# legend-exp/dspeed

Measured on AMD Instinct MI355X. Metric: waveforms/sec, 4096-sample fp32 trap-energy chain, higher is better.
Workload: dtype f32; 1 GPU; 1000000 x 4096 float32 rows per GPU, fused bl_subtract->pole_zero(tau=1716.28)->trap_filter(625,188)->fixed_time_pickoff('l'); BASELINE configs[1]; rows_per_gpu=1000000, wf_len=4096, device= (gfx950:sramecc+:xnack-), entry=build_processing_chain, kernel=dsp_energy_rr_kernel, lds_bytes_per_wave=19696, waves_per_block=4, blocks=512

## Files before the change

### dspeed_amd/csrc/dsp_energy.hip

```cpp
#include <hip/hip_runtime.h>

#include "dsp_program.h"
#include "dsp_wave.h"

struct EnergyArgs {
    const void* wf;
    int64_t wf_stride;
    int32_t wf_offset;
    int32_t len;
    const float* bl;
    int64_t bl_stride;
    float bl_const;
    int32_t has_bl;
    const float* tp;
    int64_t tp_stride;
    float tp_const;
    int32_t mode;
    float* out;
    int64_t out_stride;
    double c;
    double rr, ll;
    int32_t tau_nan;
    int32_t all_nan;
    int32_t C, pitch;
// ... 258 lines not shown
                        if (t + 2 * G3 < C) fetch(a0, a1, a2, a3, t + 2 * G3);
                        body(b0, b1, b2, b3, t + G3);
                    }
                }
                PHASE(4)
                const double D = (double)y - (double)g;
                const double delta = wave_exscan_add(D) - (double)g;
                float w4[4];
#pragma unroll
                for (int k = 0; k < 4; ++k) {
                    const float v = (float)((double)capv[k] + delta);
                    w4[k] = cl[k] >= 0 ? readlane(v, cl[k]) : 0.0f;
                }
                int fc = 0;
                result = pickoff_eval(t_in, A.mode, len, w4, fc);
                if (fc) report(fc, row);
            }
        }
        if (lane == 0) A.out[row * A.out_stride] = result;
        wave_sync();
        PHASE(5)
    }
    if (stamps && lane == 0) {
#pragma unroll
        for (int i = 0; i < 6; ++i) atomicAdd(reinterpret_cast<unsigned long long*>(err + 4) + i, tsum[i]);
    }
}

struct EnergyPlan {
    int32_t shift[3][4];
    int32_t cs[3][4];
    int32_t local[3][4];
};

__device__ __attribute__((noinline)) double rr_decay(double tau) { return exp(-1.0 / tau); }

template <int NPF, int KIND, int S, int IN, bool TAU = false>
__global__ void __launch_bounds__(256, NPF >= 32 ? 1 : 2) dsp_energy_rr_kernel(EnergyArgs A, EnergyPlan PL, int64_t n_wf, int* err) {
    extern __shared__ __attribute__((aligned(16))) unsigned char smem_raw[];
    constexpr int C = 4 * NPF + 1, len = 256 * NPF, NG = (C - 1) / 8, CS = (C - 1) / S, NGS = CS / 8;
    constexpr int BS = CS >= 16 ? 16 : CS;
    static_assert((C - 1) % (8 * S) == 0, "sub-chain length must be a whole number of 8-sample groups");
    const int lane = lane_id();
    const double inv_rr = 1.0 / A.rr, inv_ll = 1.0 / A.ll;
    const int wave = __builtin_amdgcn_readfirstlane((int)(threadIdx.x >> 6)), wpb = (int)(blockDim.x >> 6);
    float* lds = reinterpret_cast<float*>(smem_raw) + (size_t)wave * A.lds_elems_per_wave;
    for (int e = lane; e < A.lds_elems_per_wave; e += 64) lds[e] = 0.0f;
    wave_sync();
    float* slot = lds + A.slot_off;
    float* mine = slot + lane * C;
    constexpr int AUXP = NG + 1 <= 9 ? 9 : ((NG + 1) | 1);
    static_assert(NG + 1 <= AUXP && S * NGS + 1 <= AUXP && (AUXP & 1) == 1, "side array too small");
    float* aux = slot + 64 * C + 16 + lane * AUXP;
    const float* lagp[3];
#pragma unroll
    for (int k = 0; k < 3; ++k) {
        const int pos0 = lane * C - A.q[k];
        lagp[k] = (pos0 >= -C) ? slot + pos0 : slot - (2 * C + 8);
    }

    const int64_t stride_rows = (int64_t)gridDim.x * wpb;
    int64_t row = (int64_t)blockIdx.x * wpb + wave;
    typedef float f4 __attribute__((ext_vector_type(4)));
    typedef unsigned int u4 __attribute__((ext_vector_type(4)));
    constexpr int NLD = IN == 0 ? NPF : NPF / 2;
    static_assert(IN == 0 || NPF % 2 == 0, "16-bit rows: an even number of 4-sample groups per lane");
    u4 pf[NLD];
    float pf_bl = 0.0f, pf_tp = 0.0f;
    auto prefetch = [&](int64_t r) {
        const char* g = (const char*)A.wf + (r * A.wf_stride + A.wf_offset) * (IN == 0 ? 4 : 2);
#pragma unroll
        for (int b = 0; b < NLD; ++b) pf[b] = reinterpret_cast<const u4*>(g)[b * 64 + lane];
        typedef const __attribute__((address_space(1))) float* gptr;
        pf_bl = A.bl ? ((gptr)A.bl)[r * A.bl_stride] : A.bl_const;
        pf_tp = A.tp ? ((gptr)A.tp)[r * A.tp_stride] : A.tp_const;
    };
    auto report = [&](int code, int64_t r) {
        if (lane == 0 && atomicCAS(&err[0], 0, code) == 0) {
            err[1] = (int)(r & 0xffffffffll);
            err[2] = (int)(r >> 32);
        }
    };
    if (row < n_wf) prefetch(row);
    const bool stamps = (ABLATE(A) & 8) != 0;
    unsigned long long tsum[6] = {0, 0, 0, 0, 0, 0}, tlast = stamps ? stamp() : 0;
    float pend_result = 0.0f;
    int64_t pend_row = -1;

    for (; row < n_wf; row += stride_rows) {
#pragma unroll
        for (int b = 0; b < NLD; ++b) {
            if (IN == 0) {
                f4 v;
#pragma unroll
                for (int m = 0; m < 4; ++m) v[m] = __uint_as_float(pf[b][m]);
                *reinterpret_cast<f4*>(slot + (b * 64 + lane) * 4) = v - pf_bl;
            } else {
                f4 lo, hi;
#pragma unroll
                for (int m = 0; m < 4; ++m) {
                    const unsigned int wv = pf[b][m];
                    const float s0 = IN == 1 ? (float)(short)(wv & 0xffffu) : (float)(wv & 0xffffu);
                    const float s1 = IN == 1 ? (float)(short)(wv >> 16) : (float)(wv >> 16);
                    if (m < 2) {
                        lo[2 * m] = s0;
                        lo[2 * m + 1] = s1;
                    } else {
                        hi[2 * (m - 2)] = s0;
                        hi[2 * (m - 2) + 1] = s1;
                    }
                }
                *reinterpret_cast<f4*>(slot + (b * 64 + lane) * 8) = lo - pf_bl;
                *reinterpret_cast<f4*>(slot + (b * 64 + lane) * 8 + 4) = hi - pf_bl;
            }
        }
        slot[len + lane] = 0.0f;
        const float t_in = __int_as_float(__builtin_amdgcn_readfirstlane(__float_as_int(pf_tp)));
        const int64_t next = row + stride_rows;
        __builtin_amdgcn_sched_barrier(0);
        if (next < n_wf) prefetch(next);
        if (pend_row >= 0 && lane == 0) A.out[pend_row * A.out_stride] = pend_result;
        __builtin_amdgcn_sched_barrier(0);
        wave_sync();
        PHASE(0)
        RR_PRIO_AT(0)

        float result = quiet_nan<float>();
        float xr[C];
#pragma unroll
        for (int t = 0; t < C; ++t) xr[t] = mine[t];
        const float xprev = (lane > 0) ? mine[-1] : 0.0f;
        double Xp[4] = {0.0, 0.0, 0.0, 0.0};
#pragma unroll
        for (int t = 0; t < C; ++t) {
            if ((t & 7) == 0) __builtin_amdgcn_sched_barrier(0);
            Xp[t & 3] += (double)xr[t];
        }
        const double X = (Xp[0] + Xp[1]) + (Xp[2] + Xp[3]);
        double c_row = A.c;
        bool in_nan = A.tau_nan != 0;
        if constexpr (TAU) {
            const float tau = A.tau[row * A.tau_stride];
            in_nan = tau != tau;
            c_row = rr_decay((double)tau);
        }
        if (wave_any(!(fabs(X) <= 1.7976931348623157e308))) {
            bool n = false;
#pragma unroll
            for (int t = 0; t < C; ++t) n |= (xr[t] != xr[t]);
            in_nan |= wave_any(n);
        }
        PHASE(1)
        RR_PRIO_AT(1)
#pragma unroll
        for (int t = 0; t < C; ++t) asm volatile("" : "+v"(xr[t]));
        if (!in_nan) {
            const double E = wave_exscan_add(X);
            const double c = c_row;
            double xp = (double)xprev, acc = E - c * (E - xp);
            float run = 0.0f;
#pragma unroll
            for (int t = 0; t < C; ++t) {
                if ((t & 7) == 0) __builtin_amdgcn_sched_barrier(0);
                const double x = (double)xr[t];
                acc += __builtin_fma(-c, xp, x);
                const float y = (float)acc;
                xr[t] = y;
                mine[t] = y;
                xp = x;
                run += y;
                if ((t & 7) == 7) aux[t >> 3] = run;
            }
            wave_sync();
            PHASE(2)
        RR_PRIO_AT(2)
            bool pz_nan = false;
            if (wave_any(!(fabsf(run) <= 3.4028234663852886e38f))) {
                bool n = false;
#pragma unroll
                for (int t = 0; t < C; ++t) n |= (xr[t] != xr[t]);
                pz_nan = wave_any(n);
            }
            if (pz_nan) {
                report(DSP_E_PZ_NAN, row);
            } else if (!A.all_nan && !(ABLATE(A) & 4) && pickoff_in_range(t_in, len)) {
                const double Ep = wave_exscan_add((double)run);
                float g[S], y[S];
#pragma unroll
                for (int s = 0; s < S; ++s) {
                    double Ak[3];
                    float pbase[3], pv[3][8];
                    int pn[3];
#pragma unroll
                    for (int k = 0; k < 3; ++k) {
                        int r = PL.cs[k][s] * CS + PL.local[k][s];
                        asm volatile("" : "+s"(r));
                        const int gi = (r > 0 ? r - 1 : 0) >> 3;
                        pn[k] = r - 8 * gi;
                        const float b = aux[gi > 0 ? gi - 1 : 0];
                        pbase[k] = gi > 0 ? b : 0.0f;
                        const float* p = mine + 8 * gi;
#pragma unroll
                        for (int u = 0; u < 8; ++u) pv[k][u] = p[u];
                    }
#pragma unroll
                    for (int k = 0; k < 3; ++k) {
                        float part = 0.0f;
#pragma unroll
                        for (int u = 0; u < 8; ++u) part += (u < pn[k]) ? pv[k][u] : 0.0f;
                        Ak[k] = wave_shift_up(Ep + (double)(pbase[k] + part), PL.shift[k][s]);
                    }
                    const double own = Ep + (s ? (double)aux[s * NGS - 1] : 0.0);
                    double Gd;
                    if (KIND == TRAP_FILTER)
                        Gd = ((own - Ak[0]) - Ak[1]) + Ak[2];
                    else if (KIND == TRAP_NORM)
                        Gd = (((own - Ak[0]) - Ak[1]) + Ak[2]) / A.rr;
                    else
                        Gd = (own - Ak[0]) / A.rr - (Ak[1] - Ak[2]) / A.ll;
                    g[s] = (lane == 0 && s == 0) ? -0.0f : (float)Gd;
                    y[s] = g[s];
                }
                PHASE(3)
        RR_PRIO_AT(3)
                wave_sync();
                const int i0 = (int)t_in;
                int capst[2], capoff[2], caplane[2];
#pragma unroll
                for (int k = 0; k < 2; ++k) {
                    const int e = i0 + k;
                    const bool ok = e >= 0 && e < len;
                    caplane[k] = ok ? e / C : 0;
                    capoff[k] = ok ? e - caplane[k] * C : 0;
                    capst[k] = ok ? capoff[k] / BS : -1;
                }
                int capmask = (capst[0] >= 0 ? 1 << capst[0] : 0) | (capst[1] >= 0 ? 1 << capst[1] : 0);
                asm volatile("" : "+s"(capmask));
                float* capbuf = slot + 64 * C + 16 + 64 * AUXP;
                float ysb[S][BS];
                constexpr int GL = 4, NL = CS / GL;
                constexpr int PD = S == 1 ? 2 : 1;
                float lb[PD + 1][S][GL][3], lodd[3] = {0.0f, 0.0f, 0.0f};
#pragma unroll
                for (int p = 0; p < PD; ++p)
#pragma unroll
                    for (int s = 0; s < S; ++s)
#pragma unroll
                        for (int u = 0; u < GL; ++u)
#pragma unroll
                            for (int k = 0; k < 3; ++k) lb[p][s][u][k] = lagp[k][s * CS + p * GL + u];
#pragma unroll
                for (int gl = 0; gl < NL; ++gl) {
                    __builtin_amdgcn_sched_barrier(0);
                    if (gl + PD < NL) {
#pragma unroll
                        for (int s = 0; s < S; ++s)
#pragma unroll
                            for (int u = 0; u < GL; ++u)
#pragma unroll
                                for (int k = 0; k < 3; ++k) lb[(gl + PD) % (PD + 1)][s][u][k] = lagp[k][s * CS + (gl + PD) * GL + u];
                    } else if (gl + PD == NL) {
#pragma unroll
                        for (int k = 0; k < 3; ++k) lodd[k] = lagp[k][C - 1];
                    }
                    if ((gl * GL) % 8 == 0) {
#pragma unroll
                        for (int s = 0; s < S; ++s) aux[s * NGS + (gl * GL) / 8] = y[s];
                    }
                    __builtin_amdgcn_sched_barrier(0);
#pragma unroll
                    for (int u = 0; u < GL; ++u)
#pragma unroll
                        for (int s = 0; s < S; ++s) {
                            y[s] = trap_step_r<float, KIND>(y[s], xr[s * CS + gl * GL + u], lb[gl % (PD + 1)][s][u][0], lb[gl % (PD + 1)][s][u][1],
                                                          lb[gl % (PD + 1)][s][u][2], A.rr, A.ll, inv_rr, inv_ll);
                            ysb[s][(gl * GL + u) % BS] = y[s];
                        }
                    if (((gl + 1) * GL) % BS == 0) {
#pragma unroll
                        for (int s = 0; s < S; ++s) {
                            const int q = s * (CS / BS) + (gl * GL) / BS;
                            if (capmask & (1 << q)) {
#pragma unroll
                                for (int k = 0; k < 2; ++k)
                                    if (capst[k] == q && lane == caplane[k]) {
#pragma unroll
                                        for (int u = 0; u < BS; ++u) capbuf[k * 16 + u] = ysb[s][u];
                                    }
                            }
                        }
                    }
                }
                aux[S * NGS] = y[S - 1];
                y[S - 1] = trap_step_r<float, KIND>(y[S - 1], xr[C - 1], lodd[0], lodd[1], lodd[2], A.rr, A.ll, inv_rr, inv_ll);
                PHASE(4)
        RR_PRIO_AT(4)
                double D[S], Dbefore[S], Dtot = 0.0;
#pragma unroll
                for (int s = 0; s < S; ++s) {
                    D[s] = (double)y[s] - (double)g[s];
                    Dbefore[s] = Dtot;
                    Dtot += D[s];
                }
                const double T0 = wave_exscan_add(Dtot);
                const bool wide = (A.mode == 'h');
                float w4[4];
#pragma unroll
                for (int k = 0; k < 2; ++k) {
                    float v = capbuf[k * 16 + (capoff[k] % BS)];
                    v = capoff[k] == C - 1 ? y[S - 1] : v;
                    double delta = T0 - (double)g[0];
#pragma unroll
                    for (int s = 1; s < S; ++s)
                        if (capoff[k] >= s * CS) delta = (T0 + Dbefore[s]) - (double)g[s];
                    w4[1 + k] = capst[k] >= 0 ? readlane((float)((double)v + delta), caplane[k]) : 0.0f;
                }
#pragma unroll
                for (int k = 0; k < 4; k += 3) {
                    const int e = i0 - 1 + k;
                    const bool need = wide && e >= 0 && e < len;
                    w4[k] = 0.0f;
                    __builtin_amdgcn_sched_barrier(0);
                    if (need) {
                        const int l = e / C, off = e - l * C;
                        int ch = off / CS;
                        if (ch > S - 1) ch = S - 1;
                        const int loc = off - ch * CS;
                        const int gi = loc >> 3, u0 = loc & 7;
                        float ys = aux[ch * NGS + gi], gsel = 0.0f;
                        double dsel = 0.0;
#pragma unroll
                        for (int s = 0; s < S; ++s)
                            if (ch == s) {
                                gsel = g[s];
                                dsel = Dbefore[s];
                            }
                        const int base = ch * CS + gi * 8;
                        float yk = ys;
#pragma unroll
                        for (int u = 0; u < 8; ++u) {
                            const int tt = base + u;
                            ys = trap_step_r<float, KIND>(ys, mine[tt], lagp[0][tt], lagp[1][tt], lagp[2][tt], A.rr, A.ll, inv_rr, inv_ll);
                            if (u == u0) yk = ys;
                        }
                        const double delta = (T0 + dsel) - (double)gsel;
                        w4[k] = readlane((float)((double)yk + delta), l);
                    }
                }
                int fc = 0;
                result = pickoff_eval(t_in, A.mode, len, w4, fc);
                if (fc) report(fc, row);
            }
        }
        pend_result = result;
        pend_row = row;
        wave_sync();
        PHASE(5)
        RR_PRIO_AT(5)
    }
    if (pend_row >= 0 && lane == 0) A.out[pend_row * A.out_stride] = pend_result;
    if (stamps && lane == 0) {
#pragma unroll
        for (int i = 0; i < 6; ++i) atomicAdd(reinterpret_cast<unsigned long long*>(err + 4) + i, tsum[i]);
    }
}

template <int KIND, int S, int IN, bool TAU = false>
int launch_rr_kind(const EnergyArgs& A, const EnergyPlan& PL, int npf, int64_t n_wf, int* err, int blocks, int threads, int lds_bytes,
                   hipStream_t st) {
    switch (npf) {
        case 4: hipLaunchKernelGGL((dsp_energy_rr_kernel<4, KIND, S, IN, TAU>), dim3(blocks), dim3(threads), lds_bytes, st, A, PL, n_wf, err); break;
        case 8: hipLaunchKernelGGL((dsp_energy_rr_kernel<8, KIND, S, IN, TAU>), dim3(blocks), dim3(threads), lds_bytes, st, A, PL, n_wf, err); break;
        case 16: hipLaunchKernelGGL((dsp_energy_rr_kernel<16, KIND, S, IN, TAU>), dim3(blocks), dim3(threads), lds_bytes, st, A, PL, n_wf, err); break;
        case 32:
            if (S != 1) return (int)hipErrorInvalidValue;
            hipLaunchKernelGGL((dsp_energy_rr_kernel<32, KIND, 1, IN, TAU>), dim3(blocks), dim3(threads), lds_bytes, st, A, PL, n_wf, err);
            break;
        default: return (int)hipErrorInvalidValue;
    }
    return (int)hipGetLastError();
}

template <int KIND>
int launch_kind(const EnergyArgs& A, int npf, int64_t n_wf, int* err, int blocks, int threads, int lds_bytes, hipStream_t s) {
    switch (npf) {
        case 4: hipLaunchKernelGGL((dsp_energy_kernel<4, KIND>), dim3(blocks), dim3(threads), lds_bytes, s, A, n_wf, err); break;
        case 8: hipLaunchKernelGGL((dsp_energy_kernel<8, KIND>), dim3(blocks), dim3(threads), lds_bytes, s, A, n_wf, err); break;
        case 16: hipLaunchKernelGGL((dsp_energy_kernel<16, KIND>), dim3(blocks), dim3(threads), lds_bytes, s, A, n_wf, err); break;
        case 32: hipLaunchKernelGGL((dsp_energy_kernel<32, KIND>), dim3(blocks), dim3(threads), lds_bytes, s, A, n_wf, err); break;
        default: return (int)hipErrorInvalidValue;
    }
    return (int)hipGetLastError();
}

}

extern "C" int dsp_internal_launch_energy(const EnergyArgs* A, int trap_opcode, int npf, int64_t n_wf, int* err, int blocks,
                                          int threads, int lds_bytes, hipStream_t stream) {
    if (trap_opcode == DSP_OP_TRAP_FILTER) return launch_kind<TRAP_FILTER>(*A, npf, n_wf, err, blocks, threads, lds_bytes, stream);
    if (trap_opcode == DSP_OP_TRAP_NORM) return launch_kind<TRAP_NORM>(*A, npf, n_wf, err, blocks, threads, lds_bytes, stream);
    return launch_kind<TRAP_ASYM>(*A, npf, n_wf, err, blocks, threads, lds_bytes, stream);
}

extern "C" int dsp_internal_set_energy_lds(int trap_opcode, int npf, int lds_bytes) {
#define SET_(NPF, KIND)                                                                                                   \
    if (npf == NPF && kind == KIND)                                                                                        \
        return (int)hipFuncSetAttribute(reinterpret_cast<const void*>(&dsp_energy_kernel<NPF, KIND>),                      \
                                        hipFuncAttributeMaxDynamicSharedMemorySize, lds_bytes);
    const int kind = trap_opcode == DSP_OP_TRAP_FILTER ? TRAP_FILTER : (trap_opcode == DSP_OP_TRAP_NORM ? TRAP_NORM : TRAP_ASYM);
    SET_(4, TRAP_FILTER) SET_(8, TRAP_FILTER) SET_(16, TRAP_FILTER) SET_(32, TRAP_FILTER)
    SET_(4, TRAP_NORM) SET_(8, TRAP_NORM) SET_(16, TRAP_NORM) SET_(32, TRAP_NORM)
    SET_(4, TRAP_ASYM) SET_(8, TRAP_ASYM) SET_(16, TRAP_ASYM) SET_(32, TRAP_ASYM)
#undef SET_
    return (int)hipErrorInvalidValue;
}

extern "C" int dsp_internal_launch_energy_rr(const EnergyArgs* A, const EnergyPlan* PL, int trap_opcode, int npf, int S, int wf_dtype,
                                             int64_t n_wf, int* err, int blocks, int threads, int lds_bytes, hipStream_t stream) {
#define GO_(KIND)                                                                                                          \
    if (A->tau && wf_dtype == DSP_I16) return launch_rr_kind<KIND, 1, 1, true>(*A, *PL, npf, n_wf, err, blocks, threads, lds_bytes, stream); \
    if (A->tau && wf_dtype == DSP_U16) return launch_rr_kind<KIND, 1, 2, true>(*A, *PL, npf, n_wf, err, blocks, threads, lds_bytes, stream); \
    if (A->tau) return launch_rr_kind<KIND, 1, 0, true>(*A, *PL, npf, n_wf, err, blocks, threads, lds_bytes, stream);       \
    if (wf_dtype == DSP_I16) return launch_rr_kind<KIND, 1, 1>(*A, *PL, npf, n_wf, err, blocks, threads, lds_bytes, stream); \
    if (wf_dtype == DSP_U16) return launch_rr_kind<KIND, 1, 2>(*A, *PL, npf, n_wf, err, blocks, threads, lds_bytes, stream); \
    return S == 2 ? launch_rr_kind<KIND, 2, 0>(*A, *PL, npf, n_wf, err, blocks, threads, lds_bytes, stream)                \
                  : launch_rr_kind<KIND, 1, 0>(*A, *PL, npf, n_wf, err, blocks, threads, lds_bytes, stream);
    if (trap_opcode == DSP_OP_TRAP_FILTER) { GO_(TRAP_FILTER) }
    if (trap_opcode == DSP_OP_TRAP_NORM) { GO_(TRAP_NORM) }
    GO_(TRAP_ASYM)
#undef GO_
}
extern "C" const char* dsp_internal_energy_rr_kernel_name() { return "dsp_energy_rr_kernel"; }

extern "C" const char* dsp_internal_energy_kernel_name() { return "dsp_energy_kernel"; }
```

### dspeed_amd/csrc/dsp_host.cpp

```cpp
#include <hip/hip_runtime.h>

#include <execinfo.h>
#include <signal.h>
#include <unistd.h>

#include <algorithm>
#include <cmath>
#include <cstdarg>
#include <cstdio>
#include <cstdlib>
#include <cstring>
#include <map>
#include <memory>
#include <mutex>
#include <string>
#include <vector>

#include "dsp_plan.h"

extern "C" int dsp_internal_launch_vm_f32(const DevProgram* dev_prog, const IoPtrs* ptrs, int64_t n_wf, int* err, int blocks,
                                          int threads, int lds_bytes, int with_fir, int team, hipStream_t stream);
extern "C" int dsp_internal_launch_vm_f64(const DevProgram* dev_prog, const IoPtrs* ptrs, int64_t n_wf, int* err, int blocks,
                                          int threads, int lds_bytes, int with_fir, hipStream_t stream);
extern "C" int dsp_internal_set_vm_lds(int lds_bytes);
extern "C" const char* dsp_internal_vm_kernel_name();
extern "C" int dsp_internal_launch_stream_read(const void* src, int64_t bytes, uint32_t* sink, int blocks, hipStream_t stream);
extern "C" int dsp_internal_launch_fit_rows(const FitArgs* A, int wf_dtype, int compute_dtype, hipStream_t stream);
extern "C" int dsp_internal_launch_synth(void* wf, int out_dtype, int64_t n_wf, int wf_len, int64_t row_stride, float* baseline,
                                         float* t_pick, uint64_t seed, int64_t first_row, float tau, float sigma, float pick_offset,
                                         float bl_lo, float bl_hi, float amp_lo, float amp_hi, float rise_lo, float rise_hi, hipStream_t stream);

extern "C" int dsp_internal_launch_energy(const EnergyArgs* A, int trap_opcode, int npf, int64_t n_wf, int* err, int blocks,
                                          int threads, int lds_bytes, hipStream_t stream);
extern "C" int dsp_internal_set_energy_lds(int trap_opcode, int npf, int lds_bytes);
extern "C" const char* dsp_internal_energy_kernel_name();
extern "C" int dsp_internal_launch_energy_rr(const EnergyArgs* A, const EnergyPlan* PL, int trap_opcode, int npf, int S, int wf_dtype,
                                             int64_t n_wf, int* err, int blocks, int threads, int lds_bytes, hipStream_t stream);
extern "C" const char* dsp_internal_energy_rr_kernel_name();
extern "C" int dsp_internal_launch_rows(const RowsArgs* A, int64_t n_wf, int* err, int lds_bytes, hipStream_t stream);
extern "C" int dsp_internal_set_rows_lds(int lds_bytes);
extern "C" const char* dsp_internal_rows_kernel_name();
extern "C" int dsp_internal_launch_pz_rows(const PzArgs* A, int64_t n_wf, int* err, hipStream_t stream);
extern "C" const char* dsp_internal_pz_rows_kernel_name();
extern "C" int dsp_internal_launch_reduce(const ReduceArgs* A, int64_t n_wf, int dtype, int vec, int* err, hipStream_t stream);
extern "C" const char* dsp_internal_reduce_kernel_name();
extern "C" int dsp_internal_launch_scalar(const DevProgram* dev_prog, const IoPtrs* ptrs, int64_t n_wf, int n_sregs, int type, hipStream_t stream);
extern "C" int dsp_internal_set_scalar_lds(int lds_bytes);
extern "C" const char* dsp_internal_scalar_kernel_name();
extern "C" int dsp_internal_current_lds_bytes(int ma_len);
extern "C" int dsp_internal_launch_fir_runs(const FirRunsArgs* A, FirRunsTable* table, int64_t n_wf, int blocks, int* err, hipStream_t stream);
extern "C" int dsp_internal_launch_current(const CurrentArgs* A, int64_t n_wf, int blocks, int lds_bytes, hipStream_t stream);
extern "C" int dsp_internal_set_current_lds(int lds_bytes);
extern "C" const char* dsp_internal_current_kernel_name();
extern "C" int dsp_internal_fir_mfma_lds_bytes(int kend);
extern "C" int dsp_internal_launch_fir_mfma(const FirArgs* A, int64_t n_wf, int lds_bytes, hipStream_t stream);
extern "C" int dsp_internal_launch_fir_f16(const FirArgs* A, const FirF16Taps* T, int64_t n_wf, int lds_bytes, hipStream_t stream);
extern "C" int dsp_internal_fir_f16_tz(int kend);
extern "C" size_t dsp_internal_fir_f16_taps_bytes(int kend);
extern "C" int dsp_internal_fir_f16_lds_bytes();
extern "C" int dsp_internal_set_fir_f16_lds(int lds_bytes);
extern "C" const char* dsp_internal_fir_f16_kernel_name();
extern "C" int dsp_internal_set_fir_mfma_lds(int lds_bytes);
extern "C" const char* dsp_internal_fir_mfma_kernel_name();
extern "C" int dsp_internal_fir_store_lds_bytes(int kend);
extern "C" int dsp_internal_launch_fir_store(const FirArgs* A, int64_t n_wf, int lds_bytes, hipStream_t stream);
extern "C" int dsp_internal_set_fir_store_lds(int lds_bytes);
extern "C" const char* dsp_internal_fir_store_kernel_name();

#define fail dsp_fail
// ... 580 lines not shown
        }
        hipError_t e = (hipError_t)(ch->fir_f16 ? dsp_internal_launch_fir_f16(&A, &ch->f16, n_wf, dsp_internal_fir_f16_lds_bytes(), (hipStream_t)stream)
                                    : A.store   ? dsp_internal_launch_fir_store(&A, n_wf, ch->fir_lds_bytes, (hipStream_t)stream)
                                                : dsp_internal_launch_fir_mfma(&A, n_wf, ch->fir_lds_bytes, (hipStream_t)stream));
        if (e != hipSuccess) return fail(DSP_ERR_HIP, "FIR kernel launch failed: %s", hipGetErrorString(e));
        return post_err(ch, stream);
    }
    if (rows_applies(ch, io_ptrs)) {
        RowsArgs A = ch->rows;
        A.wf = io_ptrs[ch->rio_wf];
        A.bl = (const float*)at(ch->rio_bl);
        A.thr = (const float*)at(ch->rio_thr);
        A.ts = (const float*)at(ch->rio_ts);
        for (int k = 0; k < 4; ++k) A.out_mm[k] = at(ch->rio_mm[k]);
        A.out_tpt = at(ch->rio_tpt);
        A.dwt_out = at(ch->rio_dwt);
        hipError_t e = (hipError_t)dsp_internal_launch_rows(&A, n_wf, ch->dev_err, ch->rows_lds_bytes, (hipStream_t)stream);
        if (e != hipSuccess) return fail(DSP_ERR_HIP, "rows kernel launch failed: %s", hipGetErrorString(e));
        return post_err(ch, stream);
    }
    const int blocks = vm_blocks(ch, n_wf);
    const int threads = 64 * ch->waves_per_block;
    const int lds = ch->lds_bytes_per_wave * ch->waves_per_block;
    if (ch->rr_ok && ch->fused_on && ch->variant != 1 && ((reinterpret_cast<uintptr_t>(io_ptrs[ch->io_wf]) & 15u) == 0)) {
        EnergyArgs F = ch->rr;
        F.wf = io_ptrs[ch->io_wf];
        F.bl = (const float*)at(ch->io_bl);
        F.tp = (const float*)at(ch->io_tp);
        F.tau = (const float*)at(ch->io_tau);
        F.out = (float*)at(ch->io_out);
        const int S = (ch->variant == 8 && ch->wf_dtype == DSP_F32) ? 2 : 1;
        int rwpb, rblocks;
        rr_geometry(ch, n_wf, &rwpb, &rblocks);
        hipError_t e = (hipError_t)dsp_internal_launch_energy_rr(&F, &ch->plan[S - 1], ch->fused_trap, ch->fused_npf, S, ch->wf_dtype, n_wf,
                                                                 ch->dev_err, rblocks, 64 * rwpb, ch->rr_lds_bytes * rwpb, (hipStream_t)stream);
        if (e != hipSuccess) return fail(DSP_ERR_HIP, "energy kernel launch failed: %s", hipGetErrorString(e));
        return post_err(ch, stream);
    }
    if (ch->fused_ok && ch->fused_on && ((reinterpret_cast<uintptr_t>(io_ptrs[ch->io_wf]) & 15u) == 0)) {
        EnergyArgs F = ch->fused;
        F.wf = io_ptrs[ch->io_wf];
        F.bl = (const float*)at(ch->io_bl);
        F.tp = (const float*)at(ch->io_tp);
        F.out = (float*)at(ch->io_out);
        const int cw = ch->classic_wpb;
        hipError_t e = (hipError_t)dsp_internal_launch_energy(&F, ch->fused_trap, ch->fused_npf, n_wf, ch->dev_err, chain_blocks(ch, n_wf, cw, 8),
                                                              64 * cw, ch->lds_bytes_per_wave * cw, (hipStream_t)stream);
        if (e != hipSuccess) return fail(DSP_ERR_HIP, "energy kernel launch failed: %s", hipGetErrorString(e));
        return post_err(ch, stream);
    }
    hipError_t e = ch->f64 ? (hipError_t)dsp_internal_launch_vm_f64(ch->dev, &ptrs, n_wf, ch->dev_err, blocks, threads, lds, ch->has_fir,
                                                                    (hipStream_t)stream)
                           : (hipError_t)dsp_internal_launch_vm_f32(ch->dev, &ptrs, n_wf, ch->dev_err, blocks, threads * ch->host.team, lds, ch->has_fir,
                                                                    ch->host.team, (hipStream_t)stream);
    if (e != hipSuccess) return fail(DSP_ERR_HIP, "kernel launch failed: %s", hipGetErrorString(e));
    return post_err(ch, stream);
}

int dsp_chain_check(dsp_chain* ch, void* stream, int64_t* row) {
    if (!ch) return fail(DSP_ERR_ARG, "null chain");
    HIP_TRY(hipStreamSynchronize((hipStream_t)stream));
    int host_err[DSP_ERR_WORDS] = {0};
    if (ch->err_mirror) {
        memcpy(host_err, ch->err_mirror, 4 * sizeof(int));
    } else {
        HIP_TRY(staged_d2h(host_err, ch->dev_err, sizeof host_err));
    }
// ... 645 lines not shown
```

### dspeed_amd/csrc/dsp_plan.cpp

```cpp
#include "dsp_plan.h"

#include <algorithm>
#include <cmath>
#include <cstdarg>
#include <cstdio>
#include <cstdlib>
#include <cstring>
#include <memory>
#include <vector>

namespace {
thread_local std::string g_last_error;
}

int dsp_fail(int code, const char* fmt, ...) {
    char buf[512];
    va_list ap;
    va_start(ap, fmt);
    vsnprintf(buf, sizeof buf, fmt, ap);
    va_end(ap);
    g_last_error = buf;
    return code;
}
void dsp_set_last_error(const char* text) { g_last_error = text ? text : ""; }
// ... 741 lines not shown
        case DSP_OP_BL_SUBTRACT:
        case DSP_OP_MIN_MAX_NORM:
        case DSP_OP_POLE_ZERO:
        case DSP_OP_DOUBLE_POLE_ZERO:
        case DSP_OP_TRAP_FILTER:
        case DSP_OP_TRAP_NORM:
        case DSP_OP_ASYM_TRAP:
        case DSP_OP_COPY:
        case DSP_OP_WINDOWER:
        case DSP_OP_AVG_CURRENT:
        case DSP_OP_UPSAMPLER:
        case DSP_OP_CONVOLVE: out[0] = o.src; out[1] = o.dst; return 2;
        case DSP_OP_DWT_HAAR: out[0] = o.src; out[1] = o.dst; out[2] = o.ip[2]; return 3;
        case DSP_OP_MOVING_WINDOW_MULTI:
            out[0] = o.src;
            out[1] = o.dst;
            if (o.ip[1] > 1 || o.ip[3] == 1) {
                out[2] = o.ip[2];
                return 3;
            }
            return 2;
        case DSP_OP_ELEMENTWISE: {
            int n = 0;
            out[n++] = o.dst;
            if (o.src >= 0) out[n++] = o.src;
            if (o.ip[1] >= 0) out[n++] = o.ip[1];
            if (o.ip[2] >= 0) out[n++] = o.ip[2];
            return n;
        }
        default: return 0;
    }
}


int dsp_plan_build(ChainPlan* ch, const dsp_op* ops, int n_ops, const dsp_io_desc* io, int n_io, const int32_t* slot_len, int n_slots,
                   int n_sregs, int compute_dtype) {
    if (!ops || !ch || n_ops <= 0 || n_ops > DSP_MAX_OPS) return fail(DSP_ERR_ARG, "n_ops=%d out of range (1..%d)", n_ops, DSP_MAX_OPS);
    if (n_io < 0 || n_io > DSP_MAX_IO) return fail(DSP_ERR_ARG, "n_io=%d out of range", n_io);
    if (n_slots < 0 || n_slots > DSP_MAX_SLOTS) return fail(DSP_ERR_ARG, "n_slots=%d out of range", n_slots);
    if (n_sregs < 0 || n_sregs > DSP_MAX_SREGS) return fail(DSP_ERR_ARG, "n_sregs=%d out of range", n_sregs);
    if (compute_dtype != DSP_F32 && compute_dtype != DSP_F64 && compute_dtype != DSP_I64)
        return fail(DSP_ERR_ARG, "compute_dtype must be DSP_F32, DSP_F64 or DSP_I64");
    const bool i64 = compute_dtype == DSP_I64;
    const int esz = compute_dtype == DSP_F32 ? 4 : 8;
    const bool f64 = compute_dtype == DSP_F64;
    if (i64) {
        if (n_slots != 0) return fail(DSP_ERR_ARG, "an integer program (DSP_I64) has no waveform slots");
        for (int i = 0; i < n_ops; ++i)
            if (ops[i].opcode != DSP_OP_SCALAR_FUNC && ops[i].opcode != DSP_OP_STORE_SCALAR)
                return fail(DSP_ERR_ARG, "op %d: an integer program (DSP_I64) holds SCALAR_FUNC and STORE_SCALAR ops only", i);
    }

    DevProgram& P = ch->host;
    P.n_ops = n_ops;
    P.n_slots = n_slots;
    P.n_io = n_io;
    P.n_sregs = n_sregs;
    ch->f64 = f64;
    ch->i64 = i64;

    bool linear[DSP_MAX_SLOTS] = {false};
    for (int s = 0; s < n_slots; ++s) {
        bool fir_in = false, only_plain = true;
        for (int i = 0; i < n_ops; ++i) {
            const dsp_op& o = ops[i];
            int touched[4];
// ... 516 lines not shown
            if (const char* ab = getenv("DSPEED_HIP_ABLATE")) F.ablate = atoi(ab);
#endif
            ch->io_wf = ld->io;
            ch->io_out = st->io;
            ch->fused_trap = tp->ip[3];
            ch->fused_npf = slot_len[0] / 256;
            ch->fused_ok = slot_len[0] <= 4096 && wdt == DSP_F32 && !tau_col;
            if (tau_col) {
                ch->io_tau = pz->sp[0].index;
                F.tau_stride = io[ch->io_tau].row_stride;
            }
            ch->wf_dtype = wdt;
            const char* env = getenv("DSPEED_HIP_NO_FUSED");
            ch->fused_on = !(env && env[0] == '1');
            {
                EnergyArgs& I = ch->rr;
                I = F;
                const int Ci = slot_len[0] / 64 + 1;
                I.C = Ci;
                I.pitch = Ci;
                I.invC = 1.0f / (float)Ci;
                int guard = 2 * Ci + 8;
                guard = ((guard + 3) / 4) * 4;
                I.slot_off = guard;
                const int ng1 = (Ci - 1) / 8 + 1, auxp = ng1 <= 9 ? 9 : (ng1 | 1);
                int elems = guard + 64 * Ci + 16 + 64 * auxp + 32;
                elems = ((elems + 3) / 4) * 4;
                I.lds_elems_per_wave = elems;
                ch->rr_lds_bytes = elems * 4;
                for (int k = 0; k < 3; ++k) {
                    I.q[k] = dtp.ic[k];
                    I.rho[k] = 0;
                }
                for (int S = 1; S <= 2; ++S) {
                    const int CS = (Ci - 1) / S;
                    for (int k = 0; k < 3; ++k)
                        for (int sidx = 0; sidx < S; ++sidx) {
                            const int pos = sidx * CS - dtp.ic[k];
                            const int r = ((pos % Ci) + Ci) % Ci;
                            const int shift = (r - pos) / Ci;
                            int cs = r / CS;
                            if (cs > S - 1) cs = S - 1;
                            ch->plan[S - 1].shift[k][sidx] = shift;
                            ch->plan[S - 1].cs[k][sidx] = cs;
                            ch->plan[S - 1].local[k][sidx] = r - cs * CS;
                        }
                }
                ch->rr_ok = true;
                ch->variant = 6;
                if (const char* venv = getenv("DSPEED_HIP_VARIANT")) ch->variant = atoi(venv);
                if (ch->variant != 1 && ch->variant != 8) ch->variant = 6;
            }
        }
    }

    ch->fir_ok = match_fir_shape(ch, ops, n_ops, io, slot_len, n_slots, f64);
    if (!ch->fir_ok) {
        for (int k = 0; k < DSP_FIR_MAXK; ++k) ch->fio_taps[k] = ch->fio_out[k] = -1;
        ch->fir_ok = match_fir_store_shape(ch, ops, n_ops, io, slot_len, n_slots, f64);
    }
    if (ch->fir_ok) {
        const char* env = getenv("DSPEED_HIP_NO_FUSED");
        ch->fused_on = !(env && env[0] == '1');
        const char* f32 = getenv("DSPEED_HIP_FIR_F32");
        const dsp_io_desc& w = io[ch->fio_wf];
        const int es = w.dtype == DSP_F32 ? 4 : 2;
        const int n_slice = ch->fir.n;
        if (!(f32 && f32[0] == '1') && (w.row_stride * es) % 16 == 0 && (w.offset * es) % 16 == 0 &&
            ((n_slice & 7) == 0 || w.offset + ((n_slice + 7) & ~7) <= w.row_stride)) {
            ch->fir_f16 = true;
            ch->f16.tz = dsp_internal_fir_f16_tz(ch->fir.kend);
        }
    }
    ch->rows_ok = match_rows_shape(ch, ops, n_ops, io, n_io, slot_len, n_slots, dev_index, f64);
    if (!ch->rows_ok) {
        ch->rio_wf = ch->rio_bl = ch->rio_thr = ch->rio_ts = ch->rio_tpt = ch->rio_dwt = -1;
        for (int k = 0; k < 4; ++k) ch->rio_mm[k] = -1;
    } else {
        const char* env = getenv("DSPEED_HIP_NO_FUSED");
        ch->fused_on = !(env && env[0] == '1');
// ... 278 lines not shown
```

### dspeed_amd/csrc/dsp_plan.h

```cpp
#pragma once
#include <stddef.h>
#include <stdint.h>

#include <string>

#include "dsp_program.h"

constexpr int LDS_BYTES_PER_CU = 160 * 1024;

struct EnergyArgs {
    const void* wf;
    int64_t wf_stride;
    int32_t wf_offset;
    int32_t len;
    const float* bl;
    int64_t bl_stride;
    float bl_const;
    int32_t has_bl;
    const float* tp;
    int64_t tp_stride;
    float tp_const;
    int32_t mode;
    float* out;
    int64_t out_stride;
    double c;
    double rr, ll;
    int32_t tau_nan;
    int32_t all_nan;
    int32_t C, pitch;
    float invC;
    int32_t q[3], rho[3];
    int32_t lds_elems_per_wave;
    int32_t slot_off;
    const float* tau;
    int64_t tau_stride;
    int32_t ablate;
};

struct EnergyPlan {
    int32_t shift[3][4];
    int32_t cs[3][4];
    int32_t local[3][4];
};

extern "C" int dsp_internal_current_lds_bytes(int ma_len);
extern "C" int dsp_internal_fir_mfma_lds_bytes(int kend);
extern "C" int dsp_internal_fir_store_lds_bytes(int kend);
extern "C" int dsp_internal_fir_f16_tz(int kend);
extern "C" size_t dsp_internal_fir_f16_taps_bytes(int kend);
extern "C" int dsp_internal_fir_f16_lds_bytes();
extern "C" const char* dsp_internal_vm_kernel_name();
extern "C" const char* dsp_internal_energy_kernel_name();
extern "C" const char* dsp_internal_energy_rr_kernel_name();
extern "C" const char* dsp_internal_rows_kernel_name();
extern "C" const char* dsp_internal_pz_rows_kernel_name();
extern "C" const char* dsp_internal_reduce_kernel_name();
extern "C" const char* dsp_internal_scalar_kernel_name();
extern "C" const char* dsp_internal_current_kernel_name();
extern "C" const char* dsp_internal_fir_f16_kernel_name();
extern "C" const char* dsp_internal_fir_mfma_kernel_name();
extern "C" const char* dsp_internal_fir_store_kernel_name();
extern "C" const char* dsp_internal_fir_runs_kernel_name();
extern "C" int dsp_internal_fir_runs_lds_bytes(int m);

int dsp_fail(int code, const char* fmt, ...) __attribute__((format(printf, 2, 3)));
void dsp_set_last_error(const char* text);
const char* dsp_plan_last_error();
int dsp_elem_size(int dtype);

struct ChainPlan {
    DevProgram host{};
    int lds_bytes_per_wave = 0;
    int waves_per_block = 0;
    int classic_wpb = 0;
    bool has_fir = false;
    bool f64 = false;
    bool i64 = false;
    bool fused_ok = false, fused_on = true;
    EnergyArgs fused{};
    int fused_trap = 0, fused_npf = 0, wf_dtype = DSP_F32;
    bool rr_ok = false;
    int variant = 1;
    EnergyArgs rr{};
    EnergyPlan plan[2]{};
    int rr_lds_bytes = 0;
    int io_wf = -1, io_bl = -1, io_tp = -1, io_out = -1, io_tau = -1;
    bool rows_ok = false;
    RowsArgs rows{};
    int rows_lds_bytes = 0;
    int rio_wf = -1, rio_bl = -1, rio_thr = -1, rio_ts = -1, rio_mm[4] = {-1, -1, -1, -1}, rio_tpt = -1, rio_dwt = -1;
    bool fir_ok = false;
    FirArgs fir{};
    int fir_lds_bytes = 0;
    int fio_wf = -1, fio_bl = -1, fio_taps[DSP_FIR_MAXK] = {-1, -1, -1, -1}, fio_out[DSP_FIR_MAXK] = {-1, -1, -1, -1};
    bool fir_f16 = false;
    FirF16Taps f16{};
    std::string note;
    bool scalar_ok = false;
    bool cur_ok = false;
    CurrentArgs cur{};
    int cur_lds_bytes = 0, cio_wf = -1, cio_t0 = -1, cio_out[4] = {-1, -1, -1, -1};
    bool pz_ok = false;
    PzArgs pz{};
    int pio_wf = -1, pio_bl = -1, pio_out = -1, pio_tau = -1, pio_mm[4] = {-1, -1, -1, -1};
    bool red_ok = false;
    ReduceArgs red{};
    int dio_wf = -1, dio_out[5] = {-1, -1, -1, -1, -1}, dio_pick[DSP_REDUCE_PICKS] = {-1, -1, -1, -1}, red_dtype = DSP_F32;
    int dio_walk[DSP_REDUCE_WALKS] = {-1, -1, -1, -1, -1, -1}, dio_walk_thr[DSP_REDUCE_WALKS] = {-1, -1, -1, -1, -1, -1},
        dio_walk_ts[DSP_REDUCE_WALKS] = {-1, -1, -1, -1, -1, -1};
    bool red_vec = false;
    bool runs_ok = false;
    FirRunsArgs runs{};
    int uio_wf = -1, uio_taps = -1, uio_out = -1;
    int32_t slot_base[DSP_MAX_SLOTS] = {0}, slot_foot[DSP_MAX_SLOTS] = {0}, slot_first_op[DSP_MAX_SLOTS] = {0}, slot_last_op[DSP_MAX_SLOTS] = {0};
    uint8_t slot_shares[DSP_MAX_SLOTS] = {0};
};

// ... 4 lines not shown
```

### dspeed_amd/csrc/dsp_program.h

```cpp
#pragma once
#include <stdint.h>

#include "../../include/dspeed_hip.h"

#define DSP_WAVE 64
#define DSP_FC 40
#define DSP_OP_INTERNAL_NOP 101
#define DSP_OP_INTERNAL_STORES 102
#define DSP_OP_INTERNAL_ZERO 100
#define DSP_SCRATCH_ELEMS 128
#define DSP_IC 12

struct DevSlot {
    int32_t off;
    int32_t len;
    int32_t C;
    int32_t pitch;
    float invC;
    int32_t padw;
    int32_t zero_below, zero_above;
};

struct DevIO {
    int32_t kind, dtype, len, offset;
// ... 188 lines not shown
    const void* row_scale;
    const void* row_flags;
    int32_t rows_done;
    int32_t pad_;
};


#define DSP_FIR_RUNS_MAX 24
#define DSP_FIR_RUNS_MAX_TAPS 512
#define DSP_FIR_RUNS_GROUP 8
struct FirRunsTable {
    int32_t n_break;
    int32_t taps_nan;
    int32_t t[DSP_FIR_RUNS_MAX + 2];
    double weight[DSP_FIR_RUNS_MAX + 2];
    int32_t n_groups, pad_;
    int32_t first[DSP_FIR_RUNS_MAX + 2], count[DSP_FIR_RUNS_MAX + 2];
};

struct FirRunsArgs {
    const float* wf;
    int64_t wf_stride;
    int32_t wf_offset, n;
    const float* taps;
    int32_t m, p;
    int32_t start;
    int32_t keep;
    float* out;
    int64_t out_stride;
    const FirRunsTable* table;
    int32_t has_red, pad_;
    ReduceArgs red;
};
```

Measured before the change: 336.8 million waveforms/s.

## Process only the waveform prefix needed by the pickoff via chunk-size classes

Splits the per-lane chunk into up to four size classes and picks, per row, the smallest class that still covers the fixed-time pickoff index. Only that prefix of the waveform goes through the scatter, pole-zero and trap-filter stages, with per-class capture plans precomputed on the host. When the unprocessed tail holds large or non-finite values, the row falls back to the full-length path. The aim is to cut LDS traffic and recursive compute for samples after the pickoff, at the price of several kernel instantiations, more code size and branching.

```diff
diff --git a/dspeed_amd/csrc/dsp_energy.hip b/dspeed_amd/csrc/dsp_energy.hip
--- a/dspeed_amd/csrc/dsp_energy.hip
+++ b/dspeed_amd/csrc/dsp_energy.hip
@@ -314,15 +314,23 @@
     int32_t cs[3][4];
     int32_t local[3][4];
 };
+struct EnergyPlans {
+    EnergyPlan p[4];
+};
+template <int V>
+struct IntC {
+    static constexpr int value = V;
+};
 
 __device__ __attribute__((noinline)) double rr_decay(double tau) { return exp(-1.0 / tau); }
 
 template <int NPF, int KIND, int S, int IN, bool TAU = false>
-__global__ void __launch_bounds__(256, NPF >= 32 ? 1 : 2) dsp_energy_rr_kernel(EnergyArgs A, EnergyPlan PL, int64_t n_wf, int* err) {
+__global__ void __launch_bounds__(256, NPF >= 32 ? 1 : 2) dsp_energy_rr_kernel(EnergyArgs A, EnergyPlans PLS, int64_t n_wf, int* err) {
     extern __shared__ __attribute__((aligned(16))) unsigned char smem_raw[];
-    constexpr int C = 4 * NPF + 1, len = 256 * NPF, NG = (C - 1) / 8, CS = (C - 1) / S, NGS = CS / 8;
-    constexpr int BS = CS >= 16 ? 16 : CS;
-    static_assert((C - 1) % (8 * S) == 0, "sub-chain length must be a whole number of 8-sample groups");
+    constexpr int C = 4 * NPF + 1, len = 256 * NPF, NG = (C - 1) / 8;
+    constexpr int Q = S == 1 ? rr_chunk_quantum(C) : C - 1, NCLS = (C - 1) / Q;
+    static_assert(NCLS >= 1 && NCLS <= 4 && NCLS * Q == C - 1, "chunk classes must tile the lane chunk");
+    constexpr int KMIN = S == 1 ? rr_chunk_min_class(C) : 1;
     const int lane = lane_id();
     const double inv_rr = 1.0 / A.rr, inv_ll = 1.0 / A.ll;
     const int wave = __builtin_amdgcn_readfirstlane((int)(threadIdx.x >> 6)), wpb = (int)(blockDim.x >> 6);
@@ -330,16 +338,9 @@
     for (int e = lane; e < A.lds_elems_per_wave; e += 64) lds[e] = 0.0f;
     wave_sync();
     float* slot = lds + A.slot_off;
-    float* mine = slot + lane * C;
     constexpr int AUXP = NG + 1 <= 9 ? 9 : ((NG + 1) | 1);
-    static_assert(NG + 1 <= AUXP && S * NGS + 1 <= AUXP && (AUXP & 1) == 1, "side array too small");
+    static_assert(NG + 1 <= AUXP && S * ((C - 1) / S / 8) + 1 <= AUXP && (AUXP & 1) == 1, "side array too small");
     float* aux = slot + 64 * C + 16 + lane * AUXP;
-    const float* lagp[3];
-#pragma unroll
-    for (int k = 0; k < 3; ++k) {
-        const int pos0 = lane * C - A.q[k];
-        lagp[k] = (pos0 >= -C) ? slot + pos0 : slot - (2 * C + 8);
-    }
 
     const int64_t stride_rows = (int64_t)gridDim.x * wpb;
     int64_t row = (int64_t)blockIdx.x * wpb + wave;
@@ -369,9 +370,39 @@
     float pend_result = 0.0f;
     int64_t pend_row = -1;
 
-    for (; row < n_wf; row += stride_rows) {
-#pragma unroll
-        for (int b = 0; b < NLD; ++b) {
+    float t_in = 0.0f;
+    auto do_row = [&](auto cr_tag) __attribute__((always_inline)) -> bool {
+        constexpr int CR = decltype(cr_tag)::value, CS = (CR - 1) / S, NGS = CS / 8;
+        constexpr int BS = CS >= 16 ? 16 : CS;
+        static_assert((CR - 1) % (8 * S) == 0, "sub-chain length must be a whole number of 8-sample groups");
+        static_assert(CR <= C && (CR & 1) == 1, "odd lane stride: conflict-free");
+        int pcls = (CR - 1) / Q - 1;
+        asm volatile("" : "+s"(pcls));
+        const EnergyPlan& PL = PLS.p[pcls];
+        if constexpr (IN == 0 && CR < C) {
+            int mx = __float_as_int(pf_bl);
+            unsigned int mu = __float_as_uint(pf_bl);
+#pragma unroll
+            for (int b = CR / 4; b < NLD; ++b)
+#pragma unroll
+                for (int m = 0; m < 4; ++m) {
+                    mx = max(mx, (int)pf[b][m]);
+                    mu = max(mu, pf[b][m]);
+                }
+            if (wave_any(mx >= 0x7e800000 || mu >= 0xfe800000u)) return true;
+        }
+        int lane_r = lane;
+        asm volatile("" : "+v"(lane_r));
+        float* mine = slot + lane_r * CR;
+        const float* lagp[3];
+#pragma unroll
+        for (int k = 0; k < 3; ++k) {
+            const int pos0 = lane_r * CR - A.q[k];
+            lagp[k] = (pos0 >= -C) ? slot + pos0 : slot - (2 * C + 8);
+        }
+        constexpr int NST = IN == 0 ? (CR + 3) / 4 : (CR + 7) / 8;
+#pragma unroll
+        for (int b = 0; b < (NST < NLD ? NST : NLD); ++b) {
             if (IN == 0) {
                 f4 v;
 #pragma unroll
@@ -396,8 +427,7 @@
                 *reinterpret_cast<f4*>(slot + (b * 64 + lane) * 8 + 4) = hi - pf_bl;
             }
         }
-        slot[len + lane] = 0.0f;
-        const float t_in = __int_as_float(__builtin_amdgcn_readfirstlane(__float_as_int(pf_tp)));
+        if (CR == C) slot[len + lane] = 0.0f;
         const int64_t next = row + stride_rows;
         __builtin_amdgcn_sched_barrier(0);
         if (next < n_wf) prefetch(next);
@@ -408,13 +438,13 @@
         RR_PRIO_AT(0)
 
         float result = quiet_nan<float>();
-        float xr[C];
-#pragma unroll
-        for (int t = 0; t < C; ++t) xr[t] = mine[t];
+        float xr[CR];
+#pragma unroll
+        for (int t = 0; t < CR; ++t) xr[t] = mine[t];
         const float xprev = (lane > 0) ? mine[-1] : 0.0f;
         double Xp[4] = {0.0, 0.0, 0.0, 0.0};
 #pragma unroll
-        for (int t = 0; t < C; ++t) {
+        for (int t = 0; t < CR; ++t) {
             if ((t & 7) == 0) __builtin_amdgcn_sched_barrier(0);
             Xp[t & 3] += (double)xr[t];
         }
@@ -429,20 +459,20 @@
         if (wave_any(!(fabs(X) <= 1.7976931348623157e308))) {
             bool n = false;
 #pragma unroll
-            for (int t = 0; t < C; ++t) n |= (xr[t] != xr[t]);
+            for (int t = 0; t < CR; ++t) n |= (xr[t] != xr[t]);
             in_nan |= wave_any(n);
         }
         PHASE(1)
         RR_PRIO_AT(1)
 #pragma unroll
-        for (int t = 0; t < C; ++t) asm volatile("" : "+v"(xr[t]));
+        for (int t = 0; t < CR; ++t) asm volatile("" : "+v"(xr[t]));
         if (!in_nan) {
             const double E = wave_exscan_add(X);
             const double c = c_row;
             double xp = (double)xprev, acc = E - c * (E - xp);
             float run = 0.0f;
 #pragma unroll
-            for (int t = 0; t < C; ++t) {
+            for (int t = 0; t < CR; ++t) {
                 if ((t & 7) == 0) __builtin_amdgcn_sched_barrier(0);
                 const double x = (double)xr[t];
                 acc += __builtin_fma(-c, xp, x);
@@ -460,7 +490,7 @@
             if (wave_any(!(fabsf(run) <= 3.4028234663852886e38f))) {
                 bool n = false;
 #pragma unroll
-                for (int t = 0; t < C; ++t) n |= (xr[t] != xr[t]);
+                for (int t = 0; t < CR; ++t) n |= (xr[t] != xr[t]) && (CR < C || lane_r * CR + t < len);
                 pz_nan = wave_any(n);
             }
             if (pz_nan) {
@@ -512,13 +542,14 @@
                 for (int k = 0; k < 2; ++k) {
                     const int e = i0 + k;
                     const bool ok = e >= 0 && e < len;
-                    caplane[k] = ok ? e / C : 0;
-                    capoff[k] = ok ? e - caplane[k] * C : 0;
+                    caplane[k] = ok ? e / CR : 0;
+                    capoff[k] = ok ? e - caplane[k] * CR : 0;
                     capst[k] = ok ? capoff[k] / BS : -1;
                 }
                 int capmask = (capst[0] >= 0 ? 1 << capst[0] : 0) | (capst[1] >= 0 ? 1 << capst[1] : 0);
                 asm volatile("" : "+s"(capmask));
                 float* capbuf = slot + 64 * C + 16 + 64 * AUXP;
+                asm volatile("" : "+s"(capbuf));
                 float ysb[S][BS];
                 constexpr int GL = 4, NL = CS / GL;
                 constexpr int PD = S == 1 ? 2 : 1;
@@ -543,7 +574,7 @@
                                 for (int k = 0; k < 3; ++k) lb[(gl + PD) % (PD + 1)][s][u][k] = lagp[k][s * CS + (gl + PD) * GL + u];
                     } else if (gl + PD == NL) {
 #pragma unroll
-                        for (int k = 0; k < 3; ++k) lodd[k] = lagp[k][C - 1];
+                        for (int k = 0; k < 3; ++k) lodd[k] = lagp[k][CR - 1];
                     }
                     if ((gl * GL) % 8 == 0) {
 #pragma unroll
@@ -574,7 +605,7 @@
                     }
                 }
                 aux[S * NGS] = y[S - 1];
-                y[S - 1] = trap_step_r<float, KIND>(y[S - 1], xr[C - 1], lodd[0], lodd[1], lodd[2], A.rr, A.ll, inv_rr, inv_ll);
+                y[S - 1] = trap_step_r<float, KIND>(y[S - 1], xr[CR - 1], lodd[0], lodd[1], lodd[2], A.rr, A.ll, inv_rr, inv_ll);
                 PHASE(4)
         RR_PRIO_AT(4)
                 double D[S], Dbefore[S], Dtot = 0.0;
@@ -590,7 +621,7 @@
 #pragma unroll
                 for (int k = 0; k < 2; ++k) {
                     float v = capbuf[k * 16 + (capoff[k] % BS)];
-                    v = capoff[k] == C - 1 ? y[S - 1] : v;
+                    v = capoff[k] == CR - 1 ? y[S - 1] : v;
                     double delta = T0 - (double)g[0];
 #pragma unroll
                     for (int s = 1; s < S; ++s)
@@ -604,7 +635,7 @@
                     w4[k] = 0.0f;
                     __builtin_amdgcn_sched_barrier(0);
                     if (need) {
-                        const int l = e / C, off = e - l * C;
+                        const int l = e / CR, off = e - l * CR;
                         int ch = off / CS;
                         if (ch > S - 1) ch = S - 1;
                         const int loc = off - ch * CS;
@@ -639,6 +670,30 @@
         wave_sync();
         PHASE(5)
         RR_PRIO_AT(5)
+        return false;
+    };
+
+    for (; row < n_wf; row += stride_rows) {
+        t_in = __int_as_float(__builtin_amdgcn_readfirstlane(__float_as_int(pf_tp)));
+        int kcls = NCLS;
+        if constexpr (NCLS > 1) {
+            int last = 0;
+            if (!A.all_nan && pickoff_in_range(t_in, len)) last = (int)t_in + (A.mode == 'h' ? 2 : 1);
+            last = last > len - 1 ? len - 1 : last;
+            kcls = (last > 64 ? last - 64 : 0) / (64 * Q) + 1;
+            kcls = kcls < KMIN ? KMIN : kcls;
+        }
+        bool full = kcls >= NCLS;
+        if constexpr (NCLS > 1 && KMIN <= 1) {
+            if (kcls == 1) full = do_row(IntC<Q + 1>{});
+        }
+        if constexpr (NCLS > 2 && KMIN <= 2) {
+            if (kcls == 2) full = do_row(IntC<2 * Q + 1>{});
+        }
+        if constexpr (NCLS > 3 && KMIN <= 3) {
+            if (kcls == 3) full = do_row(IntC<3 * Q + 1>{});
+        }
+        if (full) do_row(IntC<C>{});
     }
     if (pend_row >= 0 && lane == 0) A.out[pend_row * A.out_stride] = pend_result;
     if (stamps && lane == 0) {
@@ -648,7 +703,7 @@
 }
 
 template <int KIND, int S, int IN, bool TAU = false>
-int launch_rr_kind(const EnergyArgs& A, const EnergyPlan& PL, int npf, int64_t n_wf, int* err, int blocks, int threads, int lds_bytes,
+int launch_rr_kind(const EnergyArgs& A, const EnergyPlans& PL, int npf, int64_t n_wf, int* err, int blocks, int threads, int lds_bytes,
                    hipStream_t st) {
     switch (npf) {
         case 4: hipLaunchKernelGGL((dsp_energy_rr_kernel<4, KIND, S, IN, TAU>), dim3(blocks), dim3(threads), lds_bytes, st, A, PL, n_wf, err); break;
@@ -697,7 +752,7 @@
     return (int)hipErrorInvalidValue;
 }
 
-extern "C" int dsp_internal_launch_energy_rr(const EnergyArgs* A, const EnergyPlan* PL, int trap_opcode, int npf, int S, int wf_dtype,
+extern "C" int dsp_internal_launch_energy_rr(const EnergyArgs* A, const EnergyPlans* PL, int trap_opcode, int npf, int S, int wf_dtype,
                                              int64_t n_wf, int* err, int blocks, int threads, int lds_bytes, hipStream_t stream) {
 #define GO_(KIND)                                                                                                          \
     if (A->tau && wf_dtype == DSP_I16) return launch_rr_kind<KIND, 1, 1, true>(*A, *PL, npf, n_wf, err, blocks, threads, lds_bytes, stream); \
diff --git a/dspeed_amd/csrc/dsp_host.cpp b/dspeed_amd/csrc/dsp_host.cpp
--- a/dspeed_amd/csrc/dsp_host.cpp
+++ b/dspeed_amd/csrc/dsp_host.cpp
@@ -34,7 +34,7 @@
                                           int threads, int lds_bytes, hipStream_t stream);
 extern "C" int dsp_internal_set_energy_lds(int trap_opcode, int npf, int lds_bytes);
 extern "C" const char* dsp_internal_energy_kernel_name();
-extern "C" int dsp_internal_launch_energy_rr(const EnergyArgs* A, const EnergyPlan* PL, int trap_opcode, int npf, int S, int wf_dtype,
+extern "C" int dsp_internal_launch_energy_rr(const EnergyArgs* A, const EnergyPlans* PL, int trap_opcode, int npf, int S, int wf_dtype,
                                              int64_t n_wf, int* err, int blocks, int threads, int lds_bytes, hipStream_t stream);
 extern "C" const char* dsp_internal_energy_rr_kernel_name();
 extern "C" int dsp_internal_launch_rows(const RowsArgs* A, int64_t n_wf, int* err, int lds_bytes, hipStream_t stream);
@@ -681,7 +681,9 @@
         const int S = (ch->variant == 8 && ch->wf_dtype == DSP_F32) ? 2 : 1;
         int rwpb, rblocks;
         rr_geometry(ch, n_wf, &rwpb, &rblocks);
-        hipError_t e = (hipError_t)dsp_internal_launch_energy_rr(&F, &ch->plan[S - 1], ch->fused_trap, ch->fused_npf, S, ch->wf_dtype, n_wf,
+        EnergyPlans plans = ch->rr_plans;
+        if (S == 2) plans.p[0] = ch->plan[1];
+        hipError_t e = (hipError_t)dsp_internal_launch_energy_rr(&F, &plans, ch->fused_trap, ch->fused_npf, S, ch->wf_dtype, n_wf,
                                                                  ch->dev_err, rblocks, 64 * rwpb, ch->rr_lds_bytes * rwpb, (hipStream_t)stream);
         if (e != hipSuccess) return fail(DSP_ERR_HIP, "energy kernel launch failed: %s", hipGetErrorString(e));
         return post_err(ch, stream);
diff --git a/dspeed_amd/csrc/dsp_plan.cpp b/dspeed_amd/csrc/dsp_plan.cpp
--- a/dspeed_amd/csrc/dsp_plan.cpp
+++ b/dspeed_amd/csrc/dsp_plan.cpp
@@ -797,6 +797,16 @@
     }
 }
 
+void rr_capture_plan(int Cr, int S, int lag, int sidx, int32_t* shift, int32_t* cs, int32_t* local) {
+    const int CS = (Cr - 1) / S;
+    const int pos = sidx * CS - lag;
+    const int r = ((pos % Cr) + Cr) % Cr;
+    int c = r / CS;
+    if (c > S - 1) c = S - 1;
+    *shift = (r - pos) / Cr;
+    *cs = c;
+    *local = r - c * CS;
+}
 
 int dsp_plan_build(ChainPlan* ch, const dsp_op* ops, int n_ops, const dsp_io_desc* io, int n_io, const int32_t* slot_len, int n_slots,
                    int n_sregs, int compute_dtype) {
@@ -1379,20 +1389,12 @@
                     I.q[k] = dtp.ic[k];
                     I.rho[k] = 0;
                 }
-                for (int S = 1; S <= 2; ++S) {
-                    const int CS = (Ci - 1) / S;
+                auto fill = [&](EnergyPlan& pl, int Cr, int S) {
                     for (int k = 0; k < 3; ++k)
-                        for (int sidx = 0; sidx < S; ++sidx) {
-                            const int pos = sidx * CS - dtp.ic[k];
-                            const int r = ((pos % Ci) + Ci) % Ci;
-                            const int shift = (r - pos) / Ci;
-                            int cs = r / CS;
-                            if (cs > S - 1) cs = S - 1;
-                            ch->plan[S - 1].shift[k][sidx] = shift;
-                            ch->plan[S - 1].cs[k][sidx] = cs;
-                            ch->plan[S - 1].local[k][sidx] = r - cs * CS;
-                        }
-                }
+                        for (int sidx = 0; sidx < S; ++sidx) rr_capture_plan(Cr, S, dtp.ic[k], sidx, &pl.shift[k][sidx], &pl.cs[k][sidx], &pl.local[k][sidx]);
+                };
+                for (int S = 1; S <= 2; ++S) fill(ch->plan[S - 1], Ci, S);
+                for (int k = 1, Qc = rr_chunk_quantum(Ci); k <= rr_chunk_classes(Ci); ++k) fill(ch->rr_plans.p[k - 1], k * Qc + 1, 1);
                 ch->rr_ok = true;
                 ch->variant = 6;
                 if (const char* venv = getenv("DSPEED_HIP_VARIANT")) ch->variant = atoi(venv);
diff --git a/dspeed_amd/csrc/dsp_plan.h b/dspeed_amd/csrc/dsp_plan.h
--- a/dspeed_amd/csrc/dsp_plan.h
+++ b/dspeed_amd/csrc/dsp_plan.h
@@ -42,6 +42,10 @@
     int32_t cs[3][4];
     int32_t local[3][4];
 };
+struct EnergyPlans {
+    EnergyPlan p[4];
+};
+void rr_capture_plan(int Cr, int S, int lag, int sidx, int32_t* shift, int32_t* cs, int32_t* local);
 
 extern "C" int dsp_internal_current_lds_bytes(int ma_len);
 extern "C" int dsp_internal_fir_mfma_lds_bytes(int kend);
@@ -83,6 +87,7 @@
     int variant = 1;
     EnergyArgs rr{};
     EnergyPlan plan[2]{};
+    EnergyPlans rr_plans{};
     int rr_lds_bytes = 0;
     int io_wf = -1, io_bl = -1, io_tp = -1, io_out = -1, io_tau = -1;
     bool rows_ok = false;
diff --git a/dspeed_amd/csrc/dsp_program.h b/dspeed_amd/csrc/dsp_program.h
--- a/dspeed_amd/csrc/dsp_program.h
+++ b/dspeed_amd/csrc/dsp_program.h
@@ -244,3 +244,7 @@
     int32_t has_red, pad_;
     ReduceArgs red;
 };
+
+constexpr int rr_chunk_quantum(int C) { return (C - 1) / 4 < 16 ? 16 : (C - 1) / 4; }
+constexpr int rr_chunk_classes(int C) { return (C - 1) / rr_chunk_quantum(C); }
+constexpr int rr_chunk_min_class(int C) { return C > 65 ? 3 : 1; }
```

Measured after the change: 352.4 million waveforms/s (median of 6 runs). +4.6%, better.
